# AnnaLew/pangenomix

Hardware: AMD Instinct MI355X
Metric: proteins/sec clustered at 0.8 identity + pan/core iters/sec, 400-genome set (higher is better)
Workload: dtype i32

## Files before the change

### pangenomix_amd/csrc/cluster.hip

```cpp
#include <algorithm>
#include <chrono>
#include <cstdlib>
#include <cmath>
#include <type_traits>
#include <functional>
#include <condition_variable>
#include <mutex>
#include <thread>
#include <vector>

#include "cluster_layout.h"
#include "cluster_tables.h"
#include "pgx_internal.h"

namespace {

using namespace pgxc;

constexpr uint32_t kWindowMax = 65536;
constexpr int kDiscoveryRounds = 2;
constexpr uint32_t kBlockCap = 4096;
constexpr uint32_t kBlockCapMin = 64;

constexpr uint32_t kMaxLen = 1u << 22;
constexpr uint32_t kPackedLenAa = 32767, kPackedLenNt = 16383;
constexpr uint32_t kSentinel = 0xFFFFFFFFu;
constexpr uint32_t kDiagLdsCap = 2048;
constexpr uint32_t kDiagLdsSmall = 512;
constexpr int kMaxBand = 64;

__constant__ int8_t kBlosum62_dev[kNAA1 * kNAA1] = PGXC_BLOSUM62_FLAT;

enum : uint32_t { F_DIAG_PASS = 1, F_BAND_OK = 2, F_ACCEPT = 4, F_TOO_BIG = 8, F_EVAL = 16, F_ALIGNED = 32 };
// ... 43 lines not shown
    const uint32_t *wcode;
    const uint16_t *wmult;
    const uint32_t *wcnt;
    const uint32_t *pk;
    const uint32_t *pk_off;
    uint32_t n_fwd;
    int32_t base;
    int32_t kd;
    int32_t nt;
    uint32_t mshift;
};
__device__ __forceinline__ uint32_t entry_rmask(const DevSeqs &S) { return (1u << S.mshift) - 1u; }
__device__ __forceinline__ uint32_t entry_fmax(const DevSeqs &S) { return 0xFFFFFFFFu >> S.mshift; }
__device__ __forceinline__ uint32_t real_of(const DevSeqs &S, uint32_t k) { return k >= S.n_fwd ? k - S.n_fwd : k; }

__constant__ int8_t kAa2Idx_dev[26] = {0, 2, 4, 3, 6, 13, 7, 8, 9, 20, 11, 10, 12,
                                       2, 20, 14, 5, 1, 15, 16, 20, 19, 17, 20, 18, 6};

__device__ __forceinline__ bool is_letter(uint8_t ch) {
    ch &= 0xDF;
    return ch >= 'A' && ch <= 'Z';
}

__global__ __launch_bounds__(256) void seq_len_kernel(const uint8_t *__restrict__ res,
                                                     const uint64_t *__restrict__ off, uint32_t n, uint64_t total,
                                                     uint32_t *__restrict__ len) {
    const uint32_t lane = threadIdx.x & 63u;
    const uint32_t i = blockIdx.x * 4u + (threadIdx.x >> 6);
    if (i >= n) return;
    const uint64_t b = off[i], e = off[i + 1];
    uint32_t c = 0;
    const uint64_t a0 = b & ~3ull;
    for (uint64_t a = a0 + 4ull * lane; a < e; a += 256) {
        uint32_t word = 0;
        if (a + 4 <= total) word = *reinterpret_cast<const uint32_t *>(res + a);
        else for (uint64_t p = a; p < total; ++p) word |= (uint32_t)res[p] << (8 * (p - a));
#pragma unroll
        for (int t = 0; t < 4; ++t) {
            const uint64_t p = a + t;
            c += (p >= b && p < e) && is_letter((uint8_t)(word >> (8 * t)));
        }
    }
    for (int d = 32; d > 0; d >>= 1) c += __shfl_xor(c, d);
    if (lane == 0) len[i] = c;
}

__global__ __launch_bounds__(256) void encode_gather_kernel(const uint8_t *__restrict__ in,
                                                           const uint64_t *__restrict__ in_off,
                                                           const uint32_t *__restrict__ order,
                                                           const uint64_t *__restrict__ out_off,
                                                           uint8_t *__restrict__ out, uint32_t n, int nt) {
    const uint32_t lane = threadIdx.x & 63u;
    const uint32_t k = blockIdx.x * 4u + (threadIdx.x >> 6);
    if (k >= n) return;
    const uint32_t src = order[k];
    const uint64_t b = in_off[src], e = in_off[src + 1];
    uint64_t w = out_off[k];
    for (uint64_t q0 = b; q0 < e; q0 += 256) {
        uint8_t chs[4];
#pragma unroll
        for (int j = 0; j < 4; ++j) { const uint64_t p = q0 + 64u * j + lane; chs[j] = p < e ? in[p] : (uint8_t)0; }
#pragma unroll
        for (int j = 0; j < 4; ++j) {
            const uint8_t ch = chs[j];
            const bool ok = is_letter(ch);
            const unsigned long long m = __ballot(ok);
            if (ok) {
                const uint8_t up = ch & 0xDF;
                const uint8_t idx = nt ? (uint8_t)(up == 'A' ? 0 : up == 'C' ? 1 : up == 'G' ? 2 : (up == 'T' || up == 'U') ? 3 : 4)
                                       : (uint8_t)kAa2Idx_dev[up - 'A'];
                out[w + __popcll(m & ((1ull << lane) - 1ull))] = idx;
            }
            w += __popcll(m);
        }
    }
}

__global__ __launch_bounds__(256) void revcomp_kernel(uint8_t *__restrict__ res, const uint64_t *__restrict__ off,
                                                     const uint32_t *__restrict__ len, uint32_t n) {
    const uint32_t lane = threadIdx.x & 63u;
    const uint32_t k = blockIdx.x * 4u + (threadIdx.x >> 6);
    if (k >= n) return;
    const uint64_t src = off[k], dst = off[n + k];
    const uint32_t L = len[k];
    for (uint32_t i = lane; i < L; i += 64) {
        const uint8_t b = res[src + L - 1 - i];
        res[dst + i] = b < 4 ? (uint8_t)(3 - b) : b;
    }
}

__global__ __launch_bounds__(256) void pack5_kernel(const uint8_t *__restrict__ res, const uint64_t *__restrict__ off,
                                                   const uint32_t *__restrict__ len,
                                                   const uint32_t *__restrict__ pk_off, uint32_t n,
                                                   uint32_t *__restrict__ pk) {
    const uint32_t lane = threadIdx.x & 63u;
    const uint32_t k = blockIdx.x * 4u + (threadIdx.x >> 6);
    if (k >= n) return;
    const uint8_t *s = res + off[k];
    const uint32_t L = len[k], nw = (L + 5u) / 6u;
    uint32_t *dst = pk + pk_off[k];
    for (uint32_t w = lane; w < nw; w += 64) {
        uint32_t x = 0;
        for (uint32_t t = 0; t < 6; ++t)
            if (6 * w + t < L) x |= (uint32_t)s[6 * w + t] << (5u * t);
        dst[w] = x;
    }
}

constexpr uint32_t kDevSortMaxLen = 65535;
constexpr uint32_t kHistLds = 4096;
constexpr uint32_t kSortShare = 1024;
constexpr uint32_t kSortCells = 4u << 20;
constexpr uint32_t kScanTile = 2048;
enum : uint32_t { H_OVER = 0, H_MAX = 1, H_BINS = 4 };

constexpr int kClearSegs = 6;
struct ClearArgs { uint32_t *p[kClearSegs]; uint32_t words[kClearSegs]; int n; uint32_t *one; };
__global__ __launch_bounds__(256) void clear_kernel(ClearArgs a) {
    const uint32_t t = blockIdx.x * 256u + threadIdx.x, step = gridDim.x * 256u;
    for (int s = 0; s < a.n; ++s)
        for (uint32_t i = t; i < a.words[s]; i += step) a.p[s][i] = 0u;
    if (a.one && t == 0) *a.one = 1u;
}

__global__ __launch_bounds__(1024) void len_hist_kernel(const uint32_t *__restrict__ len, uint32_t n, int32_t min_length,
                                                       uint32_t *__restrict__ hist) {
    __shared__ uint32_t h[kHistLds];
    for (uint32_t b = threadIdx.x; b < kHistLds; b += 1024u) h[b] = 0u;
// ... 1926 lines not shown
    S.n_input = n_in;
    if (out_n_clusters) *out_n_clusters = 0;
    const unsigned nth = host_threads(n_in);
    parallel_for(n_in, nth, [&](unsigned, size_t b, size_t e) {
        for (size_t i = b; i < e; ++i) {
            out_cluster[i] = -1; out_member[i] = -1; out_identity[i] = 0.f;
            if (out_strand) out_strand[i] = 0;
        }
    });
    if (n_in == 0) { if (stats) *stats = S; return PGX_OK; }

    DevBuf d_res(ctx, CL_SLOT_RES), d_off(ctx, CL_SLOT_OFF), d_len(ctx, CL_SLOT_LEN), d_wcode(ctx, CL_SLOT_WCODE),
        d_wmult(ctx, CL_SLOT_WMULT), d_wcnt(ctx, CL_SLOT_WCNT), d_aa1(ctx, CL_SLOT_AA1), d_aas(ctx, CL_SLOT_AAS),
        d_aan(ctx, CL_SLOT_AAN), d_lines(ctx, CL_SLOT_LINES), d_pool[2] = {{ctx, CL_SLOT_POOL0}, {ctx, CL_SLOT_POOL1}},
        d_idx(ctx, CL_SLOT_IDX), d_newbits(ctx, CL_SLOT_NEWBITS), d_touched(ctx, CL_SLOT_TOUCHED), d_first(ctx, CL_SLOT_FIRST),
        d_best_own(ctx, CL_SLOT_BEST_OWN), d_rcvis(ctx, CL_SLOT_RCVIS), d_counters(ctx, CL_SLOT_COUNTERS),
        d_visits(ctx, CL_SLOT_VISITS), d_pairsW(ctx, CL_SLOT_PAIRS_W), d_pairsK(ctx, CL_SLOT_PAIRS_K),
        d_blk_list(ctx, CL_SLOT_BLK_LIST), d_ulist(ctx, CL_SLOT_ULIST), d_new_list(ctx, CL_SLOT_NEW_LIST),
        d_flags(ctx, CL_SLOT_FLAGS), d_gscratch(ctx, CL_SLOT_GSCRATCH), d_order(ctx, CL_SLOT_ORDER), d_list(ctx, CL_SLOT_LIST),
        d_gather(ctx, CL_SLOT_GATHER), d_pk(ctx, CL_SLOT_PK), d_pkoff(ctx, CL_SLOT_PKOFF),
        d_counters2(ctx, CL_SLOT_COUNTERS2), d_best2(ctx, CL_SLOT_BEST2), d_flags2(ctx, CL_SLOT_FLAGS2),
        d_pairsW2(ctx, CL_SLOT_PAIRS_W2), d_gscratch2(ctx, CL_SLOT_GSCRATCH2),
        d_thr(ctx, CL_SLOT_THR), d_hugewords(ctx, CL_SLOT_HUGEWORDS), d_xsend(ctx, CL_SLOT_XSEND), d_xrecv(ctx, CL_SLOT_XRECV),
        d_hist(ctx, CL_SLOT_HIST), d_sortcnt(ctx, CL_SLOT_SORTCNT), d_tilesum(ctx, CL_SLOT_TILESUM), d_runs(ctx, CL_SLOT_RUNS);
    uint32_t n_codes = 1;
    for (int t = 0; t < P->word_len; ++t) n_codes *= nt ? 4u : (uint32_t)kNAA1;
    static_assert(kSegs == 4, "eight codes per word of the round's map");
    const uint32_t bm_words = (n_codes / 8 + 2 + 3) & ~3u;
    const bool overlap = !nt && !std::getenv("PGX_NO_OVERLAP");
    DevBuf d_in_len(ctx, CL_SLOT_IN_LEN);
    PGX_HIP(d_in_len.alloc((size_t)n_in * 4));
    constexpr uint32_t kHistWords = H_BINS + kDevSortMaxLen + 1;
    PGX_HIP(d_hist.alloc((size_t)kHistWords * 4));
    PGX_HIP(d_idx.alloc(16));
    PGX_HIP(d_newbits.alloc(2 * (size_t)bm_words * 4 + 16));
    PGX_HIP(d_counters.alloc(C_COUNT * 4));
    PGX_HIP(d_visits.alloc(8));
    if (overlap) PGX_HIP(d_counters2.alloc(C_COUNT * 4));
    {
        ClearArgs ca{};
        auto seg = [&](DevBuf &b, size_t words) { ca.p[ca.n] = b.as<uint32_t>(); ca.words[ca.n] = (uint32_t)words; ++ca.n; };
        seg(d_hist, kHistWords);
        seg(d_newbits, 2 * (size_t)bm_words);
        seg(d_counters, C_COUNT);
        seg(d_visits, 2);
        if (overlap) seg(d_counters2, C_COUNT);
        ca.one = d_idx.as<uint32_t>();
        clear_kernel<<<1024, 256, 0, st>>>(ca);
        LAUNCH_CHECK();
    }
    {
        ProfScope prof(ctx, "seq_len_kernel", st);
        seq_len_kernel<<<(n_in + 3) / 4, 256, 0, st>>>(d_residues, d_offsets, n_in, total_in, d_in_len.as<uint32_t>());
        len_hist_kernel<<<std::min(64u, (n_in + 1023u) / 1024u), 1024, 0, st>>>(d_in_len.as<uint32_t>(), n_in, P->min_length,
                                                                               d_hist.as<uint32_t>());
    }
    LAUNCH_CHECK();
    HostVec<uint32_t> h_hist(ctx, CL_HOST_HIST, kHistWords);
    PGX_REQUIRE(h_hist.ok(), "out of host memory");
    PGX_HIP(hipMemcpyAsync(h_hist.data(), d_hist.p, (size_t)(H_BINS + kHistLds) * 4, hipMemcpyDeviceToHost, st));
    PGX_HIP(hipStreamSynchronize(st));
    const bool dev_sort = h_hist[H_OVER] == 0 && !std::getenv("PGX_HOST_PROLOGUE");
    uint32_t max_len = h_hist[H_MAX];
    if (dev_sort && max_len >= kHistLds) {
        PGX_HIP(hipMemcpyAsync(h_hist.data() + H_BINS + kHistLds, d_hist.as<uint32_t>() + H_BINS + kHistLds,
                               (size_t)(max_len + 1 - kHistLds) * 4, hipMemcpyDeviceToHost, st));
        PGX_HIP(hipStreamSynchronize(st));
    }
    phase("  seq_len + histogram + copy");
    const uint32_t *len_hist = h_hist.data() + H_BINS;
    uint32_t n = 0;
    HostVec<uint32_t> order(ctx, CL_HOST_ORDER, dev_sort ? 0 : n_in);
    std::vector<uint32_t> host_hist;
    if (dev_sort) {
        for (uint32_t L = 0; L <= max_len; ++L) n += len_hist[L];
    } else {
// ... 179 lines not shown
        ca.p[0] = cnt; ca.words[0] = cells; ca.n = 1;
        clear_kernel<<<std::min(2048u, (cells + 255u) / 256u), 256, 0, st>>>(ca);
        sort_count_kernel<<<(n_in + 255) / 256, 256, 0, st>>>(in_len, n_in, P->min_length, max_len, per, n_shares, cnt);
        tile_sum_kernel<<<tiles, 256, 0, st>>>(cnt, cells, d_tilesum.as<uint32_t>());
        tile_scan_kernel<<<tiles, 256, 0, st>>>(cnt, cells, d_tilesum.as<uint32_t>());
        sort_place_kernel<<<(n_shares + 3) / 4, 256, 0, st>>>(in_len, n_in, P->min_length, max_len, per, n_shares, cnt, n,
                                                              d_order.as<uint32_t>());
        LAUNCH_CHECK();
        PGX_HIP(hipMemcpyAsync(order.data(), d_order.p, (size_t)n * 4, hipMemcpyDeviceToHost, st));
    } else {
        PGX_HIP(hipMemcpyAsync(d_order.p, order.data(), (size_t)n * 4, hipMemcpyHostToDevice, st));
    }
    {
        const size_t runs_bytes = 2 * ((size_t)n_runs + 1) * 8;
        PGX_HIP(d_runs.alloc(runs_bytes));
        PGX_HIP(hipMemcpyAsync(d_runs.p, h_runs.data(), runs_bytes, hipMemcpyHostToDevice, st));
        const uint64_t *const dr_off = d_runs.as<uint64_t>();
        const uint32_t *const dr_pos = reinterpret_cast<const uint32_t *>(dr_off + n_runs + 1), *const dr_pk = dr_pos + n_runs + 1;
        layout_kernel<<<nv / 256 + 1, 256, 0, st>>>(dr_off, dr_pos, dr_pk, n_runs, max_len, n, nv, d_len.as<uint32_t>(),
                                                    d_off.as<uint64_t>(), d_pkoff.as<uint32_t>());
        LAUNCH_CHECK();
    }
    {
        ProfScope prof(ctx, "encode_gather_kernel", st);
        encode_gather_kernel<<<(n + 3) / 4, 256, 0, st>>>(d_residues, d_offsets, d_order.as<uint32_t>(),
                                                          d_off.as<uint64_t>(), d_res.as<uint8_t>(), n, nt ? 1 : 0);
        if (both)
            revcomp_kernel<<<(n + 3) / 4, 256, 0, st>>>(d_res.as<uint8_t>(), d_off.as<uint64_t>(),
                                                        d_len.as<uint32_t>(), n);
        pack5_kernel<<<(nv + 3) / 4, 256, 0, st>>>(d_res.as<uint8_t>(), d_off.as<uint64_t>(), d_len.as<uint32_t>(),
                                                   d_pkoff.as<uint32_t>(), nv, d_pk.as<uint32_t>());
    }
    LAUNCH_CHECK();
    {
        PGX_HIP(d_thr.alloc(3 * ((size_t)max_len + 1) * 4));
        PGX_HIP(hipMemcpyAsync(d_thr.p, h_thr.data(), 3 * ((size_t)max_len + 1) * 4, hipMemcpyHostToDevice, st));
        thresholds_kernel<<<(n + 255) / 256, 256, 0, st>>>(d_len.as<uint32_t>(), n, d_thr.as<int32_t>(), max_len + 1,
                                                          d_aa1.as<int32_t>(), d_aas.as<int32_t>(), d_aan.as<int32_t>());
        LAUNCH_CHECK();
    }
    phase("alloc + sort + layout + encode (enq)");
    {
        const int wl = P->word_len;
        auto first_with_words_le = [&](uint32_t cap) { return pgxc::first_with_words_le(run_pos, max_len, cap, wl); };
        const uint32_t k32 = first_with_words_le(32768), k8 = first_with_words_le(8192),
                       k2 = first_with_words_le(2048), k1k = first_with_words_le(1023), k5 = first_with_words_le(512);
        int rc;
        uint8_t *r8 = d_res.as<uint8_t>(); uint64_t *o64 = d_off.as<uint64_t>(); uint32_t *l32 = d_len.as<uint32_t>();
        uint32_t *wc = d_wcode.as<uint32_t>(); uint16_t *wm = d_wmult.as<uint16_t>(); uint32_t *wn = d_wcnt.as<uint32_t>();
        const int base = nt ? 4 : kNAA1;
        for (uint32_t half = 0; half < (both ? 2u : 1u); ++half) {
            const uint32_t o = half * n;
            if (k32) {
                uint32_t slots = 65536;
// ... 34 lines not shown
    phase("host lengths + offsets");
    uint64_t max_window_words = 0;
    uint32_t max_chunks = 1;
    {
        Chunks C;
        size_t nf = 0;
        for (uint32_t b0 = 0, nbw; b0 < n; b0 += nbw) {
            while (nf < flush_at.size() && flush_at[nf] <= b0) ++nf;
            nbw = form_window(b0, C, nf < flush_at.size() ? flush_at[nf] : n);
            max_window_words = std::max<uint64_t>(max_window_words, h_off[b0 + nbw] - h_off[b0]);
            max_chunks = std::max(max_chunks, C.n);
        }
        if (!flush_at.empty())
            max_window_words = std::max<uint64_t>(max_window_words, h_off[std::min(n, window_cap)]);
    }
    if (chunking && flush_at.empty())
        max_window_words = std::max<uint64_t>(max_window_words,
            std::min<uint64_t>(h_off[std::min(n, window_cap)], (uint64_t)kMaxChunks * std::max<uint64_t>(chunk_words, max_len)));
    PGX_REQUIRE(max_window_words < 0xFFFFFFF0ull, "window too large");
    PGX_HIP(d_touched.alloc((max_window_words + 16) * sizeof(Deferred)));
    if (chunking && n > window_cap / 2) max_chunks = kMaxChunks;
    uint32_t tag_stride = 1;
    while (tag_stride < max_chunks) tag_stride *= 2;
    PGX_HIP(d_first.alloc((size_t)tag_stride * n_codes * 4 + 16));
    std::vector<uint32_t> rep_seq;
    HostVec<int32_t> cluster_of(ctx, CL_HOST_CLUSTER_OF, n, -1);
    HostVec<int32_t> iden_of(ctx, CL_HOST_IDEN_OF, n, -1);
    PGX_REQUIRE(cluster_of.ok() && iden_of.ok(), "out of host memory");
    Pinned<Pair> hW(ctx, CL_PIN_W), hK(ctx, CL_PIN_K);
    Pinned<unsigned long long> h_best(ctx, CL_PIN_BEST), h_rcvis(ctx, CL_PIN_RCVIS);
    Pinned<uint32_t> h_cnt(ctx, CL_PIN_CNT), h_blk(ctx, CL_PIN_BLK), h_new(ctx, CL_PIN_NEW), h_list(ctx, CL_PIN_LIST),
        h_push(ctx, CL_PIN_PUSH);
    Pinned<Pair> h_gather(ctx, CL_PIN_GATHER);
    constexpr uint32_t kPrefix = 65536;
    PGX_HIP(h_best.reserve(window_cap)); PGX_HIP(h_cnt.reserve(C_COUNT)); PGX_HIP(h_blk.reserve(kBlockCap));
    PGX_HIP(h_new.reserve(window_cap)); PGX_HIP(hK.reserve(pair_cap_k)); PGX_HIP(hW.reserve(kPrefix));
    PGX_HIP(h_rcvis.reserve(window_cap)); PGX_HIP(h_push.reserve(2 * (size_t)window_cap + 4 * kBlockCap));
    PGX_HIP(h_list.reserve(pair_cap_k)); PGX_HIP(h_gather.reserve(pair_cap_k));
    Pinned<Pair> hW2(ctx, CL_PIN_W2);
    Pinned<unsigned long long> h_best2(ctx, CL_PIN_BEST2);
    Pinned<uint32_t> h_ccnt(ctx, CL_PIN_CCNT), h_ccnt2(ctx, CL_PIN_CCNT2);
    PGX_HIP(h_ccnt.reserve(C_COUNT));
    if (overlap) { PGX_HIP(hW2.reserve(kPrefix)); PGX_HIP(h_best2.reserve(window_cap)); PGX_HIP(h_ccnt2.reserve(C_COUNT)); }
    struct Events {
        hipEvent_t strike[2] = {nullptr, nullptr}, post[2] = {nullptr, nullptr};
        ~Events() { for (hipEvent_t e : strike) if (e) (void)hipEventDestroy(e); for (hipEvent_t e : post) if (e) (void)hipEventDestroy(e); }
    } ev;
// ... 32 lines not shown
    uint64_t n_rounds = 0;

    uint64_t gpu_pairs = 0, gpu_aligned = 0, gpu_aligned_bytes = 0, filter_walk_words = 0;
    auto account = [&](const Pair *pp, uint32_t cnt) {
        for (uint32_t i = 0; i < cnt; ++i) {
            ++gpu_pairs;
            if ((pp[i].flags & (F_DIAG_PASS | F_BAND_OK)) != (F_DIAG_PASS | F_BAND_OK)) continue;
            ++gpu_aligned;
            gpu_aligned_bytes += h_len[pp[i].q] + h_len[pp[i].r];
        }
    };
    auto window_error = [&](uint32_t e, uint32_t at) {
        pgx_set_error("pgx_cluster_greedy: capacity failure in the window at %u%s:%s%s%s%s%s%s", at,
                      exchanging ? " (on this or another process)" : "",
                      e & E_TOUCHED ? " append scratch list full;" : "", e & E_POOL ? " overflow pool of the word index full;" : "",
                      e & E_TABLE ? " exact table of the filter overflowed;" : "",
                      e & E_BAND ? " alignment band wider than 64 diagonals;" : "", e & E_PAIRS ? " candidate pair buffer overflow;" : "",
                      e & E_WORDMULT ? " a word occurs more than 65535 times in one sequence;" : "");
    };
    const bool trace = std::getenv("PGX_TRACE") != nullptr;
    const uint32_t filter_grid = 4096u;
    uint32_t epoch_idx = 0;
    uint32_t epoch_tag = 0;
    PGX_HIP(hipMemsetAsync(d_first.p, 0, (size_t)tag_stride * n_codes * 4, st));
    phase("window set-up");
    const auto t_loop0 = std::chrono::steady_clock::now();
    double t_resolve = 0.0, t_close = 0.0;
    uint64_t n_blocks = 0;
    g_wait_s = 0.0;
    std::function<int()> deferred;
    std::vector<uint32_t> members;
    uint64_t pending_words = 0;
    Chunks chunks;
    Pinned<uint8_t> h_taken(ctx, CL_PIN_TAKEN);
    if (!flush_at.empty()) { PGX_HIP(h_taken.reserve(n)); std::fill(h_taken.p, h_taken.p + n, (uint8_t)0); }
    auto drain = [&]() -> int {
        if (deferred) { int rc = deferred(); deferred = nullptr; if (rc) return rc; }
        PGX_HIP(hipStreamSynchronize(st_main));
        PGX_HIP(hipStreamSynchronize(ctx->stream2));
        return PGX_OK;
    };
    size_t next_flush = 0;
    bool sweeping = false;
    uint32_t sweep_at = 0;
    for (uint32_t cursor = 0, nb = 0; cursor < n;) {
        if (!sweeping && next_flush < flush_at.size() && cursor == flush_at[next_flush]) {
            ++next_flush;
// ... 146 lines not shown
            LAUNCH_CHECK();
            return PGX_OK;
        };
        auto filter_new_and_evaluate = [&](const uint32_t *d_lo, const uint32_t *d_hi) -> int {
            FilterArgs F = FA;
            F.epoch = epoch_idx; F.d_round_lo = d_lo; F.d_round_hi = d_hi;
            F.newbits = d_newbits.as<uint32_t>() + (size_t)(epoch_idx & 1u) * bm_words;
            {
                ProfScope prof(ctx, "filter_kernel<new>", st);
                auto kern = nt ? filter_kernel<true, true> : filter_kernel<false, true>;
                kern<<<std::min(filter_grid, (ns + 3) / 4), 256, 0, st>>>(DS, F);
            }
            LAUNCH_CHECK();
            filter_walk_words += window_words * (both ? 2 : 1) / shard_count;
            return evaluate_round();
        };
        uint32_t n_listed = 0;
        if (sweep) { int rc = begin_host_side(); if (rc) return rc; }
        if (!sweep) {
        if (overlap && S.sweeps > 1)
            PGX_HIP(hipStreamWaitEvent(st, ev.post[set ^ 1], 0));
        static const int n_disc = std::getenv("PGX_ROUNDS") ? std::atoi(std::getenv("PGX_ROUNDS")) : kDiscoveryRounds;
        for (int round = 0; round < n_disc; ++round) {
            if (++epoch_tag == 0xFFFFu) { PGX_HIP(hipMemsetAsync(d_first.p, 0, (size_t)tag_stride * n_codes * 4, st)); epoch_tag = 1; }
            const uint32_t which = (uint32_t)round & 1u;
            uint32_t *const d_n_open = dc + (which ? C_ROUND_OPEN2 : C_ROUND_OPEN);
            list_open_kernel<<<(nb + 255) / 256, 256, 0, st>>>(d_best, d_done, b0, nb, d_ulist.as<uint32_t>(), dc, which);
            LAUNCH_CHECK();
            {
                ProfScope prof(ctx, "discover_kernels", st);
                first_open_kernel<<<std::min(2048u, (nb + 3) / 4), 256, 0, st>>>(DS, d_ulist.as<uint32_t>(), d_n_open, b0,
                                                                                 epoch_tag, d_first.as<uint32_t>(), tag_stride,
                                                                                 chunks, d_aan.as<int32_t>(), d_accepted);
                certain_kernel<<<std::min(2048u, (nb + 3) / 4), 256, 0, st>>>(DS, d_ulist.as<uint32_t>(), d_n_open, b0,
                                                                              both ? 1u : 0u, epoch_tag, d_first.as<uint32_t>(), tag_stride,
                                                                              chunks,
                                                                              d_aan.as<int32_t>(), d_accepted, d_done, d_new_list.as<uint32_t>(),
                                                                              dc + C_NEW);
            }
            LAUNCH_CHECK();
            int rc = index_append(d_new_list.as<uint32_t>(), dc + C_SEG0, dc + C_NEW);
            if (rc) return rc;
            rc = filter_new_and_evaluate(dc + C_SEG0, dc + C_NEW);
            if (rc) return rc;
        }
        bool first_block = true;
        n_listed = 0;
// ... 318 lines not shown
        unsigned long long h[16], z[16] = {0};
        PGX_HIP(hipMemcpyFromSymbol(h, HIP_SYMBOL(g_ftime), sizeof h));
        PGX_HIP(hipMemcpyToSymbol(HIP_SYMBOL(g_ftime), z, sizeof z));
        static const char *nm[12] = {"prologue", "words+probes", "compaction", "last slab", "sync+reduce", "pass2 begin",
                                     "pass2 walk", "pass2 sync", "emit", "bucket clear", "kernel end", "-"};
        double tot = 0;
        for (int i = 0; i < 12; ++i) tot += (double)h[i];
        for (int i = 0; i < 11; ++i) fprintf(stderr, "[ftime] %-14s %6.2f %%\n", nm[i], 100.0 * (double)h[i] / tot);
        fprintf(stderr, "[ftime] %llu waves, %.0f clocks per wave; direct %llu, fallbacks %llu, classic %llu\n", h[12], tot / (double)h[12], h[13], h[14], h[15]);
    }
#endif
    if (overlap) PGX_HIP(hipStreamSynchronize(ctx->stream2));
    unsigned long long visits_table = 0;
    PGX_HIP(hipMemcpyAsync(&visits_table, d_visits.p, 8, hipMemcpyDeviceToHost, st));
    PGX_HIP(hipStreamSynchronize(st));
    S.posting_visits = visits_table + visits_rc;
    S.reserved[0] = gpu_pairs; S.reserved[1] = gpu_aligned; S.reserved[2] = gpu_aligned_bytes;
    S.reserved[3] = filter_walk_words;
    S.n_clusters = rep_seq.size();

    phase("window loop");
    if (out_n_clusters) *out_n_clusters = (uint32_t)rep_seq.size();
    if (stats) *stats = S;
    return PGX_OK;
}

extern "C" int pgx_cluster_greedy(pgx_ctx *ctx, const uint8_t *residues, const uint64_t *offsets,
                                  uint32_t n_in, const pgx_cluster_params *P, int32_t *out_cluster,
                                  int32_t *out_member, float *out_identity, uint8_t *out_strand,
                                  uint32_t *out_n_clusters, pgx_cluster_stats *stats) {
    PGX_REQUIRE(ctx && P, "NULL argument");
    PGX_REQUIRE(n_in == 0 || (residues && offsets), "NULL sequence arrays");
    PGX_HIP(hipSetDevice(ctx->device_id));
    for (uint32_t i = 0; i < n_in; ++i) PGX_REQUIRE(offsets[i + 1] >= offsets[i], "offsets must be non-decreasing");
    const uint64_t total_in = n_in ? offsets[n_in] : 0;
    DevBuf d_res(ctx, CL_SLOT_UP_RES), d_off(ctx, CL_SLOT_UP_OFF);
    PGX_HIP(d_res.alloc(total_in + 16));
    PGX_HIP(d_off.alloc(((size_t)n_in + 1) * 8));
    if (n_in) {
        { int rc = pgx_staged_h2d(ctx, d_res.p, residues, total_in, ctx->stream); if (rc) return rc; }
        PGX_HIP(hipMemcpyAsync(d_off.p, offsets, ((size_t)n_in + 1) * 8, hipMemcpyHostToDevice, ctx->stream));
    }
    return pgx_cluster_greedy_dev(ctx, d_res.as<uint8_t>(), d_off.as<uint64_t>(), n_in, total_in, P, out_cluster,
                                  out_member, out_identity, out_strand, out_n_clusters, stats, ctx->stream);
}
```

### pangenomix_amd/csrc/pgx_internal.h

```cpp
#pragma once
#include <hip/hip_runtime.h>
#include <cstdarg>
#include <cstdint>
#include <cstdio>
#include <cstring>
#include "../../include/pgx.h"
#include "pgx_guard.h"
#include "pgx_pack.h"

#include <string>
#include <utility>
#include <algorithm>
#include <cstdlib>
#include <vector>

struct ProfSlot {
    std::string name;
    double total_ms = 0.0;
    uint64_t launches = 0;
    std::vector<std::pair<hipEvent_t, hipEvent_t>> pending;
};

enum DevSlot : int {
    CL_SLOT_IN_LEN = 0, CL_SLOT_RES, CL_SLOT_OFF, CL_SLOT_LEN, CL_SLOT_WCODE, CL_SLOT_WMULT, CL_SLOT_WCNT, CL_SLOT_AA1,
    CL_SLOT_AAS, CL_SLOT_AAN, CL_SLOT_LINES, CL_SLOT_POOL0, CL_SLOT_POOL1, CL_SLOT_IDX, CL_SLOT_NEWBITS, CL_SLOT_TOUCHED,
    CL_SLOT_FIRST, CL_SLOT_BEST_OWN, CL_SLOT_RCVIS, CL_SLOT_COUNTERS, CL_SLOT_VISITS, CL_SLOT_PAIRS_W, CL_SLOT_PAIRS_K,
    CL_SLOT_BLK_LIST, CL_SLOT_ULIST, CL_SLOT_NEW_LIST, CL_SLOT_FLAGS, CL_SLOT_GSCRATCH, CL_SLOT_ORDER, CL_SLOT_LIST,
    CL_SLOT_GATHER, CL_SLOT_PK, CL_SLOT_PKOFF, CL_SLOT_COUNTERS2, CL_SLOT_BEST2, CL_SLOT_FLAGS2, CL_SLOT_PAIRS_W2,
    CL_SLOT_GSCRATCH2, CL_SLOT_THR, CL_SLOT_HUGEWORDS, CL_SLOT_XSEND, CL_SLOT_XRECV, CL_SLOT_HIST, CL_SLOT_SORTCNT,
    CL_SLOT_TILESUM, CL_SLOT_RUNS, CL_SLOT_UP_RES, CL_SLOT_UP_OFF,
    PC_SLOT_ROWS, PC_SLOT_GENOMES, PC_SLOT_BITS, PC_SLOT_PERMS, PC_SLOT_PAN, PC_SLOT_CORE, PC_SLOT_WS, PC_SLOT_CNT,
    PC_SLOT_COUNTS, PC_SLOT_TABLE, PGX_SLOT_RESIDENT, PC_SLOT_RES_A, PC_SLOT_RES_B, PC_SLOT_RES_C, PC_SLOT_RES_D,
    HP_SLOT_TAB, HP_SLOT_A, HP_SLOT_K,
    PGX_SLOT_BERN_BITS, BN_SLOT_ROWS, BN_SLOT_GENOMES, BN_SLOT_CNT, BN_SLOT_MAP, BN_SLOT_PQ, BN_SLOT_OUT, BN_SLOT_WS,
    BB_SLOT_WORDS0, BB_SLOT_WORDS1, BB_SLOT_CDF, BB_SLOT_MODEL, BB_SLOT_KS, BB_SLOT_HIST, BB_SLOT_IDX,
    FC_SLOT_BITS, FC_SLOT_ROWS, FC_SLOT_GENOMES, FC_SLOT_CNT, FC_SLOT_WS, FC_SLOT_MAP, FC_SLOT_CMAP, FC_SLOT_CROWS,
    FC_SLOT_CCOLS, FC_SLOT_CLEARED,
    FC_SLOT_M_LISTS, FC_SLOT_M_WS, FC_SLOT_M_OUT, FC_SLOT_M_MATRIX,
    AS_SLOT_BITS, AS_SLOT_ROWS, AS_SLOT_GENOMES, AS_SLOT_CNT, AS_SLOT_WS, AS_SLOT_IN, AS_SLOT_OUT,
    RN_SLOT_ABITS, RN_SLOT_AROWS, RN_SLOT_AGENOMES, RN_SLOT_ACNT, RN_SLOT_GBITS, RN_SLOT_GROWS, RN_SLOT_GGENOMES,
    RN_SLOT_GCNT, RN_SLOT_IN, RN_SLOT_WS, RN_SLOT_OUT,
    CS_SLOT_WS, CS_SLOT_THR, CS_SLOT_OUT,
    SC_SLOT_TEXT, SC_SLOT_KEYS, SC_SLOT_FOUND, SC_SLOT_WS,
    CD_SLOT_INIT, CD_SLOT_TABLE, CD_SLOT_SOLVER, CD_SLOT_WS,
    DM_SLOT_KEYS, DM_SLOT_KEY_OFF, DM_SLOT_TABLE, DM_SLOT_QUERIES, DM_SLOT_QUERY_OFF, DM_SLOT_OUT,
    SD_SLOT_ROWS, SD_SLOT_GENOMES, SD_SLOT_A_BITS, SD_SLOT_A_CNT, SD_SLOT_B_BITS, SD_SLOT_B_CNT, SD_SLOT_OUT,
    SV_SLOT_BITS, SV_SLOT_ROWS, SV_SLOT_GENOMES, SV_SLOT_CNT, SV_SLOT_WS, SV_SLOT_IN, SV_SLOT_OUT,
    PX_SLOT_TEXT, PX_SLOT_WINDOWS, PX_SLOT_OUT, PX_SLOT_BLOB, PX_SLOT_RECORDS, PX_SLOT_WS, PX_SLOT_RESULT,
    AN_SLOT_TOK, AN_SLOT_OFFSETS, AN_SLOT_WS, AN_SLOT_RESULT,
    GR_SLOT_IN, GR_SLOT_WS, GR_SLOT_OUT,
    TS_SLOT_TEXT, TS_SLOT_IN, TS_SLOT_OUT,
    DEV_SLOT_COUNT
};
// ... 9 lines not shown
    SV_HOST_STATUS,
    PX_HOST_OFFSETS,
    HOST_SLOT_COUNT
};
enum PinSlot : int {
    CL_PIN_W = 0, CL_PIN_K, CL_PIN_BEST, CL_PIN_CNT, CL_PIN_BLK, CL_PIN_NEW, CL_PIN_RCVIS, CL_PIN_LIST, CL_PIN_GATHER,
    CL_PIN_PUSH, CL_PIN_W2, CL_PIN_BEST2, CL_PIN_CCNT, CL_PIN_CCNT2, CL_PIN_TAKEN,
    PIN_SLOT_COUNT
};

struct pgx_ctx {
    int device_id;
    hipStream_t stream;
    hipStream_t stream2;
    hipEvent_t ev_main = nullptr, ev_side[2] = {nullptr, nullptr};
    hipDeviceProp_t prop;
    bool profiling = false;
    std::vector<ProfSlot> prof;
    std::vector<hipEvent_t> event_pool;
    std::pair<void *, size_t> arena[DEV_SLOT_COUNT] = {};
    std::pair<void *, size_t> host_arena[PIN_SLOT_COUNT] = {};
    std::pair<void *, size_t> host_scratch[HOST_SLOT_COUNT] = {};
    std::vector<hipEvent_t> stage_events;
    uint64_t resident_token = 0, resident_next = 1;
    uint32_t resident_genes = 0, resident_genomes = 0;
    uint32_t bern_genes = 0, bern_genomes = 0;
    bool bern_loaded = false;
    uint64_t bern_cd_stats[4] = {0, 0, 0, 0};
    bool dict_loaded = false;
    uint32_t dict_keys = 0, dict_flags = 0;
    const void *dict_d_keys = nullptr, *dict_d_offsets = nullptr, *dict_d_table = nullptr;
    std::vector<int32_t> fcd_rows, fcd_cols;
    std::vector<uint64_t> fcd_row_off, fcd_col_off, fcd_left;
    void *comm = nullptr;
    int comm_rank = 0, comm_world = 0;
};

template <typename T>
struct HostVec {
    T *p = nullptr;
    size_t n = 0;
    HostVec(pgx_ctx *ctx, HostSlot slot, size_t count) { bind(ctx, slot, count); }
    HostVec(pgx_ctx *ctx, HostSlot slot, size_t count, T fill) {
        bind(ctx, slot, count);
        if (p) std::fill(p, p + n, fill);
    }
// ... 195 lines not shown
```

Before: 16.45 million.

## Fuse encode and 5-bit packing into length-bucketed SWAR kernel; cache tag epoch

Replaces the per-sequence wave-wide encode_gather and pack5 passes with a fused encode_pack kernel. It reads 16-byte chunks, encodes four residues per word through byte-permute table lookups, and writes both the byte codes and the 5-bit packed words. Sequences are split into length buckets and handled by thread groups of 64, 16 or 8, and sequences containing non-letter characters go to a slow-path list that the old kernels handle. seq_len now counts letters with SWAR over 16-thread groups. The tag buffer memset is skipped across calls by carrying the epoch tag in the context, which reuses state between calls and relies on the buffer staying untouched.

```diff
diff --git a/pangenomix_amd/csrc/cluster.hip b/pangenomix_amd/csrc/cluster.hip
--- a/pangenomix_amd/csrc/cluster.hip
+++ b/pangenomix_amd/csrc/cluster.hip
@@ -9,6 +9,7 @@
 #include <thread>
 #include <vector>
 
+#include "cluster_encode.h"
 #include "cluster_layout.h"
 #include "cluster_tables.h"
 #include "pgx_internal.h"
@@ -98,56 +99,150 @@
     return ch >= 'A' && ch <= 'Z';
 }
 
+struct Bytes16 { uint32_t w[4]; };
+struct __attribute__((packed, aligned(1))) Packed16 { uint32_t w[4]; };
+struct __attribute__((packed, aligned(1))) Packed8 { uint64_t v; };
+struct __attribute__((packed, aligned(1))) Packed4 { uint32_t v; };
+struct __attribute__((packed, aligned(1))) Packed2 { uint16_t v; };
+struct __attribute__((packed, aligned(4))) Words4 { uint32_t w[4]; };
+__device__ __forceinline__ Bytes16 load16(const uint8_t *__restrict__ in, uint64_t at, uint64_t lo, uint64_t hi) {
+    Bytes16 r;
+    if (at >= lo && at + 16 <= hi) {
+        const Packed16 x = *reinterpret_cast<const Packed16 *>(in + at);
+        r.w[0] = x.w[0]; r.w[1] = x.w[1]; r.w[2] = x.w[2]; r.w[3] = x.w[3];
+    } else {
+        r.w[0] = r.w[1] = r.w[2] = r.w[3] = 0u;
+        for (uint32_t t = 0; t < 16; ++t)
+            if (at + t >= lo && at + t < hi) r.w[t >> 2] |= (uint32_t)in[at + t] << (8u * (t & 3u));
+    }
+    return r;
+}
+
+constexpr uint32_t kLenGroup = 16;
 __global__ __launch_bounds__(256) void seq_len_kernel(const uint8_t *__restrict__ res,
                                                      const uint64_t *__restrict__ off, uint32_t n, uint64_t total,
                                                      uint32_t *__restrict__ len) {
-    const uint32_t lane = threadIdx.x & 63u;
-    const uint32_t i = blockIdx.x * 4u + (threadIdx.x >> 6);
+    const uint32_t gl = threadIdx.x & (kLenGroup - 1u);
+    const uint32_t i = (blockIdx.x * 256u + threadIdx.x) / kLenGroup;
     if (i >= n) return;
-    const uint64_t b = off[i], e = off[i + 1];
+    const uint64_t mis = reinterpret_cast<uintptr_t>(res) & 15u;
+    const uint8_t *const base = res - mis;
+    const uint64_t b = mis + off[i], e = mis + off[i + 1];
     uint32_t c = 0;
-    const uint64_t a0 = b & ~3ull;
-    for (uint64_t a = a0 + 4ull * lane; a < e; a += 256) {
-        uint32_t word = 0;
-        if (a + 4 <= total) word = *reinterpret_cast<const uint32_t *>(res + a);
-        else for (uint64_t p = a; p < total; ++p) word |= (uint32_t)res[p] << (8 * (p - a));
+    for (uint64_t a = (b & ~15ull) + 16ull * gl; a < e; a += 32ull * kLenGroup) {
+        const uint64_t a2 = a + 16ull * kLenGroup;
+        Bytes16 x = load16(base, a, mis, mis + total), y;
+        if (a2 < e) y = load16(base, a2, mis, mis + total);
+        else y.w[0] = y.w[1] = y.w[2] = y.w[3] = 0u;
+        if (b > a) drop_first(x.w, 4, (uint32_t)(b - a));
+        if (e - a < 16) keep_first(x.w, 4, (uint32_t)(e - a));
+        if (a2 < e && e - a2 < 16) keep_first(y.w, 4, (uint32_t)(e - a2));
 #pragma unroll
-        for (int t = 0; t < 4; ++t) {
-            const uint64_t p = a + t;
-            c += (p >= b && p < e) && is_letter((uint8_t)(word >> (8 * t)));
-        }
-    }
-    for (int d = 32; d > 0; d >>= 1) c += __shfl_xor(c, d);
-    if (lane == 0) len[i] = c;
+        for (int t = 0; t < 4; ++t) c += __popc(letter_bits(x.w[t])) + __popc(letter_bits(y.w[t]));
+    }
+    for (int d = kLenGroup / 2; d > 0; d >>= 1) c += __shfl_xor(c, d);
+    if (gl == 0) len[i] = c;
+}
+
+constexpr uint32_t kEncLen8 = 8u * kLaneBytes, kEncLen16 = 16u * kLaneBytes;
+template <uint32_t G>
+__global__ __launch_bounds__(256) void encode_pack_kernel(const uint8_t *__restrict__ in,
+                                                         const uint64_t *__restrict__ in_off, uint64_t total,
+                                                         const uint32_t *__restrict__ order,
+                                                         const uint64_t *__restrict__ out_off,
+                                                         const uint32_t *__restrict__ len,
+                                                         const uint32_t *__restrict__ pk_off, uint32_t k0, uint32_t k1,
+                                                         EncTable T, uint8_t *__restrict__ out,
+                                                         uint32_t *__restrict__ pk, uint32_t *__restrict__ slow) {
+    const uint32_t gl = threadIdx.x & (G - 1u);
+    const uint32_t k = k0 + (blockIdx.x * 256u + threadIdx.x) / G;
+    if (k >= k1) return;
+    const uint32_t src = order[k], L = len[k];
+    const uint64_t b = in_off[src], e = in_off[src + 1];
+    if (e - b != (uint64_t)L) {
+        if (gl == 0) slow[1u + atomicAdd(slow, 1u)] = k;
+        return;
+    }
+    uint8_t *const dst = out + out_off[k];
+    uint32_t *const dpk = pk + pk_off[k];
+    for (uint32_t p = gl * kLaneBytes; p < L; p += G * kLaneBytes) {
+        const uint32_t rem = L - p;
+        uint32_t enc[kLaneWords];
+#pragma unroll
+        for (int j = 0; j < 3; ++j) {
+            Bytes16 x;
+            if (rem > 16u * j) x = load16(in, b + p + 16u * j, 0, total);
+            else x.w[0] = x.w[1] = x.w[2] = x.w[3] = 0u;
+#pragma unroll
+            for (int t = 0; t < 4; ++t) enc[4 * j + t] = encode4(x.w[t], T);
+        }
+        if (rem < kLaneBytes) keep_first(enc, (int)kLaneWords, rem);
+#pragma unroll
+        for (int j = 0; j < 3; ++j) {
+            uint8_t *q = dst + p + 16u * j;
+            if (rem >= 16u * (j + 1)) {
+                Packed16 s;
+#pragma unroll
+                for (int t = 0; t < 4; ++t) s.w[t] = enc[4 * j + t];
+                *reinterpret_cast<Packed16 *>(q) = s;
+            } else if (rem > 16u * j) {
+                const uint32_t r = rem - 16u * j;
+                uint64_t cur = enc[4 * j] | (uint64_t)enc[4 * j + 1] << 32;
+                if (r & 8u) {
+                    reinterpret_cast<Packed8 *>(q)->v = cur;
+                    cur = enc[4 * j + 2] | (uint64_t)enc[4 * j + 3] << 32; q += 8;
+                }
+                if (r & 4u) { reinterpret_cast<Packed4 *>(q)->v = (uint32_t)cur; cur >>= 32; q += 4; }
+                if (r & 2u) { reinterpret_cast<Packed2 *>(q)->v = (uint16_t)cur; cur >>= 16; q += 2; }
+                if (r & 1u) *q = (uint8_t)cur;
+            }
+        }
+        uint32_t w[kLanePacked];
+        pack48(enc, w);
+        uint32_t *const qw = dpk + p / 6u;
+        const uint32_t nw = rem >= kLaneBytes ? kLanePacked : (rem + 5u) / 6u;
+        if (nw == kLanePacked) {
+            Words4 s0, s1;
+#pragma unroll
+            for (int t = 0; t < 4; ++t) { s0.w[t] = w[t]; s1.w[t] = w[4 + t]; }
+            *reinterpret_cast<Words4 *>(qw) = s0;
+            *reinterpret_cast<Words4 *>(qw + 4) = s1;
+        } else {
+#pragma unroll
+            for (int t = 0; t < (int)kLanePacked - 1; ++t)
+                if ((uint32_t)t < nw) qw[t] = w[t];
+        }
+    }
 }
 
 __global__ __launch_bounds__(256) void encode_gather_kernel(const uint8_t *__restrict__ in,
                                                            const uint64_t *__restrict__ in_off,
                                                            const uint32_t *__restrict__ order,
                                                            const uint64_t *__restrict__ out_off,
-                                                           uint8_t *__restrict__ out, uint32_t n, int nt) {
-    const uint32_t lane = threadIdx.x & 63u;
-    const uint32_t k = blockIdx.x * 4u + (threadIdx.x >> 6);
-    if (k >= n) return;
-    const uint32_t src = order[k];
-    const uint64_t b = in_off[src], e = in_off[src + 1];
-    uint64_t w = out_off[k];
-    for (uint64_t q0 = b; q0 < e; q0 += 256) {
-        uint8_t chs[4];
+                                                           uint8_t *__restrict__ out, const uint32_t *__restrict__ slow, int nt) {
+    const uint32_t lane = threadIdx.x & 63u, n = slow[0];
+    for (uint32_t i = blockIdx.x * 4u + (threadIdx.x >> 6); i < n; i += gridDim.x * 4u) {
+        const uint32_t k = slow[1u + i];
+        const uint32_t src = order[k];
+        const uint64_t b = in_off[src], e = in_off[src + 1];
+        uint64_t w = out_off[k];
+        for (uint64_t q0 = b; q0 < e; q0 += 256) {
+            uint8_t chs[4];
 #pragma unroll
-        for (int j = 0; j < 4; ++j) { const uint64_t p = q0 + 64u * j + lane; chs[j] = p < e ? in[p] : (uint8_t)0; }
+            for (int j = 0; j < 4; ++j) { const uint64_t p = q0 + 64u * j + lane; chs[j] = p < e ? in[p] : (uint8_t)0; }
 #pragma unroll
-        for (int j = 0; j < 4; ++j) {
-            const uint8_t ch = chs[j];
-            const bool ok = is_letter(ch);
-            const unsigned long long m = __ballot(ok);
-            if (ok) {
-                const uint8_t up = ch & 0xDF;
-                const uint8_t idx = nt ? (uint8_t)(up == 'A' ? 0 : up == 'C' ? 1 : up == 'G' ? 2 : (up == 'T' || up == 'U') ? 3 : 4)
-                                       : (uint8_t)kAa2Idx_dev[up - 'A'];
-                out[w + __popcll(m & ((1ull << lane) - 1ull))] = idx;
-            }
-            w += __popcll(m);
+            for (int j = 0; j < 4; ++j) {
+                const uint8_t ch = chs[j];
+                const bool ok = is_letter(ch);
+                const unsigned long long m = __ballot(ok);
+                if (ok) {
+                    const uint8_t up = ch & 0xDF;
+                    const uint8_t idx = nt ? (uint8_t)(up == 'A' ? 0 : up == 'C' ? 1 : up == 'G' ? 2 : (up == 'T' || up == 'U') ? 3 : 4)
+                                           : (uint8_t)kAa2Idx_dev[up - 'A'];
+                    out[w + __popcll(m & ((1ull << lane) - 1ull))] = idx;
+                }
+                w += __popcll(m);
+            }
         }
     }
 }
@@ -167,19 +262,21 @@
 
 __global__ __launch_bounds__(256) void pack5_kernel(const uint8_t *__restrict__ res, const uint64_t *__restrict__ off,
                                                    const uint32_t *__restrict__ len,
-                                                   const uint32_t *__restrict__ pk_off, uint32_t n,
-                                                   uint32_t *__restrict__ pk) {
+                                                   const uint32_t *__restrict__ pk_off, const uint32_t *__restrict__ slow,
+                                                   uint32_t k0, uint32_t n, uint32_t *__restrict__ pk) {
     const uint32_t lane = threadIdx.x & 63u;
-    const uint32_t k = blockIdx.x * 4u + (threadIdx.x >> 6);
-    if (k >= n) return;
-    const uint8_t *s = res + off[k];
-    const uint32_t L = len[k], nw = (L + 5u) / 6u;
-    uint32_t *dst = pk + pk_off[k];
-    for (uint32_t w = lane; w < nw; w += 64) {
-        uint32_t x = 0;
-        for (uint32_t t = 0; t < 6; ++t)
-            if (6 * w + t < L) x |= (uint32_t)s[6 * w + t] << (5u * t);
-        dst[w] = x;
+    if (slow) n = slow[0];
+    for (uint32_t i = blockIdx.x * 4u + (threadIdx.x >> 6); i < n; i += gridDim.x * 4u) {
+        const uint32_t k = slow ? slow[1u + i] : k0 + i;
+        const uint8_t *s = res + off[k];
+        const uint32_t L = len[k], nw = (L + 5u) / 6u;
+        uint32_t *dst = pk + pk_off[k];
+        for (uint32_t w = lane; w < nw; w += 64) {
+            uint32_t x = 0;
+            for (uint32_t t = 0; t < 6; ++t)
+                if (6 * w + t < L) x |= (uint32_t)s[6 * w + t] << (5u * t);
+            dst[w] = x;
+        }
     }
 }
 
@@ -2152,7 +2249,8 @@
         d_counters2(ctx, CL_SLOT_COUNTERS2), d_best2(ctx, CL_SLOT_BEST2), d_flags2(ctx, CL_SLOT_FLAGS2),
         d_pairsW2(ctx, CL_SLOT_PAIRS_W2), d_gscratch2(ctx, CL_SLOT_GSCRATCH2),
         d_thr(ctx, CL_SLOT_THR), d_hugewords(ctx, CL_SLOT_HUGEWORDS), d_xsend(ctx, CL_SLOT_XSEND), d_xrecv(ctx, CL_SLOT_XRECV),
-        d_hist(ctx, CL_SLOT_HIST), d_sortcnt(ctx, CL_SLOT_SORTCNT), d_tilesum(ctx, CL_SLOT_TILESUM), d_runs(ctx, CL_SLOT_RUNS);
+        d_hist(ctx, CL_SLOT_HIST), d_sortcnt(ctx, CL_SLOT_SORTCNT), d_tilesum(ctx, CL_SLOT_TILESUM), d_runs(ctx, CL_SLOT_RUNS),
+        d_slow(ctx, CL_SLOT_SLOW);
     uint32_t n_codes = 1;
     for (int t = 0; t < P->word_len; ++t) n_codes *= nt ? 4u : (uint32_t)kNAA1;
     static_assert(kSegs == 4, "eight codes per word of the round's map");
@@ -2167,6 +2265,7 @@
     PGX_HIP(d_counters.alloc(C_COUNT * 4));
     PGX_HIP(d_visits.alloc(8));
     if (overlap) PGX_HIP(d_counters2.alloc(C_COUNT * 4));
+    PGX_HIP(d_slow.alloc(((size_t)n_in + 1) * 4));
     {
         ClearArgs ca{};
         auto seg = [&](DevBuf &b, size_t words) { ca.p[ca.n] = b.as<uint32_t>(); ca.words[ca.n] = (uint32_t)words; ++ca.n; };
@@ -2175,13 +2274,14 @@
         seg(d_counters, C_COUNT);
         seg(d_visits, 2);
         if (overlap) seg(d_counters2, C_COUNT);
+        seg(d_slow, 1);
         ca.one = d_idx.as<uint32_t>();
         clear_kernel<<<1024, 256, 0, st>>>(ca);
         LAUNCH_CHECK();
     }
     {
         ProfScope prof(ctx, "seq_len_kernel", st);
-        seq_len_kernel<<<(n_in + 3) / 4, 256, 0, st>>>(d_residues, d_offsets, n_in, total_in, d_in_len.as<uint32_t>());
+        seq_len_kernel<<<(n_in + 256 / kLenGroup - 1) / (256 / kLenGroup), 256, 0, st>>>(d_residues, d_offsets, n_in, total_in, d_in_len.as<uint32_t>());
         len_hist_kernel<<<std::min(64u, (n_in + 1023u) / 1024u), 1024, 0, st>>>(d_in_len.as<uint32_t>(), n_in, P->min_length,
                                                                                d_hist.as<uint32_t>());
     }
@@ -2407,14 +2507,39 @@
         LAUNCH_CHECK();
     }
     {
-        ProfScope prof(ctx, "encode_gather_kernel", st);
-        encode_gather_kernel<<<(n + 3) / 4, 256, 0, st>>>(d_residues, d_offsets, d_order.as<uint32_t>(),
-                                                          d_off.as<uint64_t>(), d_res.as<uint8_t>(), n, nt ? 1 : 0);
-        if (both)
-            revcomp_kernel<<<(n + 3) / 4, 256, 0, st>>>(d_res.as<uint8_t>(), d_off.as<uint64_t>(),
-                                                        d_len.as<uint32_t>(), n);
-        pack5_kernel<<<(nv + 3) / 4, 256, 0, st>>>(d_res.as<uint8_t>(), d_off.as<uint64_t>(), d_len.as<uint32_t>(),
-                                                   d_pkoff.as<uint32_t>(), nv, d_pk.as<uint32_t>());
+        ProfScope prof(ctx, "encode_pack_kernel", st);
+        EncTable tab{};
+        for (uint32_t c = 0; c < 26; ++c) {
+            const char up = (char)('A' + c);
+            const uint32_t idx = nt ? (up == 'A' ? 0u : up == 'C' ? 1u : up == 'G' ? 2u : (up == 'T' || up == 'U') ? 3u : 4u)
+                                    : (uint32_t)kAa2Idx[c];
+            tab.t[c >> 2] |= idx << (8u * (c & 3u));
+        }
+        const uint32_t k16 = max_len > kEncLen16 ? run_pos[max_len - kEncLen16] : 0u, k8 = max_len > kEncLen8 ? run_pos[max_len - kEncLen8] : 0u;
+        uint8_t *const r8 = d_res.as<uint8_t>();
+        uint32_t *const pk32 = d_pk.as<uint32_t>(), *const slow = d_slow.as<uint32_t>();
+        if (k16)
+            encode_pack_kernel<64><<<(k16 + 3) / 4, 256, 0, st>>>(d_residues, d_offsets, total_in, d_order.as<uint32_t>(),
+                                                                  d_off.as<uint64_t>(), d_len.as<uint32_t>(), d_pkoff.as<uint32_t>(),
+                                                                  0u, k16, tab, r8, pk32, slow);
+        if (k8 > k16)
+            encode_pack_kernel<16><<<(k8 - k16 + 15) / 16, 256, 0, st>>>(d_residues, d_offsets, total_in, d_order.as<uint32_t>(),
+                                                                        d_off.as<uint64_t>(), d_len.as<uint32_t>(), d_pkoff.as<uint32_t>(),
+                                                                        k16, k8, tab, r8, pk32, slow);
+        if (n > k8)
+            encode_pack_kernel<8><<<(n - k8 + 31) / 32, 256, 0, st>>>(d_residues, d_offsets, total_in, d_order.as<uint32_t>(),
+                                                                     d_off.as<uint64_t>(), d_len.as<uint32_t>(), d_pkoff.as<uint32_t>(),
+                                                                     k8, n, tab, r8, pk32, slow);
+        const uint32_t slow_grid = std::min(256u, (n + 3) / 4);
+        encode_gather_kernel<<<slow_grid, 256, 0, st>>>(d_residues, d_offsets, d_order.as<uint32_t>(), d_off.as<uint64_t>(), r8,
+                                                        slow, nt ? 1 : 0);
+        if (both) {
+            revcomp_kernel<<<(n + 3) / 4, 256, 0, st>>>(r8, d_off.as<uint64_t>(), d_len.as<uint32_t>(), n);
+            pack5_kernel<<<std::min(2048u, (n + 3) / 4), 256, 0, st>>>(r8, d_off.as<uint64_t>(), d_len.as<uint32_t>(),
+                                                                       d_pkoff.as<uint32_t>(), nullptr, n, n, pk32);
+        }
+        pack5_kernel<<<slow_grid, 256, 0, st>>>(r8, d_off.as<uint64_t>(), d_len.as<uint32_t>(), d_pkoff.as<uint32_t>(), slow,
+                                                0u, 0u, pk32);
     }
     LAUNCH_CHECK();
     {
@@ -2495,7 +2620,8 @@
     if (chunking && n > window_cap / 2) max_chunks = kMaxChunks;
     uint32_t tag_stride = 1;
     while (tag_stride < max_chunks) tag_stride *= 2;
-    PGX_HIP(d_first.alloc((size_t)tag_stride * n_codes * 4 + 16));
+    const size_t tag_bytes = (size_t)tag_stride * n_codes * 4;
+    PGX_HIP(d_first.alloc(tag_bytes + 16));
     std::vector<uint32_t> rep_seq;
     HostVec<int32_t> cluster_of(ctx, CL_HOST_CLUSTER_OF, n, -1);
     HostVec<int32_t> iden_of(ctx, CL_HOST_IDEN_OF, n, -1);
@@ -2574,7 +2700,15 @@
     const uint32_t filter_grid = 4096u;
     uint32_t epoch_idx = 0;
     uint32_t epoch_tag = 0;
-    PGX_HIP(hipMemsetAsync(d_first.p, 0, (size_t)tag_stride * n_codes * 4, st));
+    {
+        const auto &slot = ctx->arena[CL_SLOT_FIRST];
+        if (ctx->cl_tag_bytes == tag_bytes && ctx->cl_tag_stride == tag_stride && ctx->cl_tag_buf == slot.first &&
+            ctx->cl_tag_cap == slot.second)
+            epoch_tag = ctx->cl_tag_epoch;
+        else
+            PGX_HIP(hipMemsetAsync(d_first.p, 0, tag_bytes, st));
+        ctx->cl_tag_bytes = 0;
+    }
     phase("window set-up");
     const auto t_loop0 = std::chrono::steady_clock::now();
     double t_resolve = 0.0, t_close = 0.0;
@@ -2767,7 +2901,7 @@
             PGX_HIP(hipStreamWaitEvent(st, ev.post[set ^ 1], 0));
         static const int n_disc = std::getenv("PGX_ROUNDS") ? std::atoi(std::getenv("PGX_ROUNDS")) : kDiscoveryRounds;
         for (int round = 0; round < n_disc; ++round) {
-            if (++epoch_tag == 0xFFFFu) { PGX_HIP(hipMemsetAsync(d_first.p, 0, (size_t)tag_stride * n_codes * 4, st)); epoch_tag = 1; }
+            if (++epoch_tag == 0xFFFFu) { PGX_HIP(hipMemsetAsync(d_first.p, 0, tag_bytes, st)); epoch_tag = 1; }
             const uint32_t which = (uint32_t)round & 1u;
             uint32_t *const d_n_open = dc + (which ? C_ROUND_OPEN2 : C_ROUND_OPEN);
             list_open_kernel<<<(nb + 255) / 256, 256, 0, st>>>(d_best, d_done, b0, nb, d_ulist.as<uint32_t>(), dc, which);
@@ -3132,6 +3266,8 @@
     phase("window loop");
     if (out_n_clusters) *out_n_clusters = (uint32_t)rep_seq.size();
     if (stats) *stats = S;
+    ctx->cl_tag_buf = ctx->arena[CL_SLOT_FIRST].first; ctx->cl_tag_cap = ctx->arena[CL_SLOT_FIRST].second;
+    ctx->cl_tag_bytes = tag_bytes; ctx->cl_tag_stride = tag_stride; ctx->cl_tag_epoch = epoch_tag;
     return PGX_OK;
 }
 
diff --git a/pangenomix_amd/csrc/cluster_encode.h b/pangenomix_amd/csrc/cluster_encode.h
--- /dev/null
+++ b/pangenomix_amd/csrc/cluster_encode.h
@@ -0,0 +1,72 @@
+#pragma once
+#include <cstdint>
+
+#if defined(__HIPCC__)
+#define PGXC_HD __attribute__((host)) __attribute__((device)) inline __attribute__((always_inline))
+#else
+#define PGXC_HD inline
+#endif
+
+namespace pgxc {
+
+constexpr uint32_t kLaneBytes = 48, kLaneWords = kLaneBytes / 4, kLanePacked = kLaneBytes / 6;
+
+PGXC_HD uint32_t letter_bits(uint32_t x) {
+    const uint32_t u = x & 0xDFDFDFDFu, t = u & 0x7F7F7F7Fu;
+    return (t + 0x3F3F3F3Fu) & ~(t + 0x25252525u) & ~u & 0x80808080u;
+}
+
+PGXC_HD uint32_t pick_bytes(uint32_t hi, uint32_t lo, uint32_t sel) {
+#if defined(__HIP_DEVICE_COMPILE__)
+    return __builtin_amdgcn_perm(hi, lo, sel);
+#else
+    const uint64_t tab = ((uint64_t)hi << 32) | lo;
+    uint32_t r = 0;
+    for (int i = 0; i < 4; ++i) r |= (uint32_t)((tab >> (8u * ((sel >> (8 * i)) & 7u))) & 0xFFu) << (8 * i);
+    return r;
+#endif
+}
+
+struct EncTable { uint32_t t[8]; };
+
+PGXC_HD uint32_t encode4(uint32_t x, const EncTable &T) {
+    const uint32_t c = (x & 0xDFDFDFDFu) - 0x41414141u;
+    const uint32_t sel = c & 0x07070707u;
+    const uint32_t by3 = ((c >> 1) & 0x04040404u) | 0x03020100u, by4 = ((c >> 2) & 0x04040404u) | 0x03020100u;
+    const uint32_t r0 = pick_bytes(T.t[1], T.t[0], sel), r1 = pick_bytes(T.t[3], T.t[2], sel);
+    const uint32_t r2 = pick_bytes(T.t[5], T.t[4], sel), r3 = pick_bytes(T.t[7], T.t[6], sel);
+    return pick_bytes(pick_bytes(r3, r2, by3), pick_bytes(r1, r0, by3), by4);
+}
+
+PGXC_HD void keep_first(uint32_t *e, int n, uint32_t rem) {
+    const uint32_t full = rem >> 2, part = (1u << (8u * (rem & 3u))) - 1u;
+#if defined(__HIP_DEVICE_COMPILE__)
+#pragma unroll
+#endif
+    for (int t = 0; t < n; ++t) e[t] = (uint32_t)t < full ? e[t] : (uint32_t)t == full ? e[t] & part : 0u;
+}
+PGXC_HD void drop_first(uint32_t *e, int n, uint32_t skip) {
+    const uint32_t full = skip >> 2, part = (1u << (8u * (skip & 3u))) - 1u;
+#if defined(__HIP_DEVICE_COMPILE__)
+#pragma unroll
+#endif
+    for (int t = 0; t < n; ++t) e[t] = (uint32_t)t < full ? 0u : (uint32_t)t == full ? e[t] & ~part : e[t];
+}
+
+PGXC_HD uint32_t squeeze4(uint32_t e) {
+    const uint32_t t = (e & 0x001F001Fu) | ((e & 0x1F001F00u) >> 3);
+    return (t & 0x3FFu) | ((t >> 6) & 0xFFC00u);
+}
+
+PGXC_HD void pack48(const uint32_t e[kLaneWords], uint32_t w[kLanePacked]) {
+#if defined(__HIP_DEVICE_COMPILE__)
+#pragma unroll
+#endif
+    for (int g = 0; g < 4; ++g) {
+        const uint32_t q0 = squeeze4(e[3 * g]), q1 = squeeze4(e[3 * g + 1]), q2 = squeeze4(e[3 * g + 2]);
+        w[2 * g] = q0 | ((q1 & 0x3FFu) << 20);
+        w[2 * g + 1] = (q1 >> 10) | (q2 << 10);
+    }
+}
+
+}
diff --git a/pangenomix_amd/csrc/pgx_internal.h b/pangenomix_amd/csrc/pgx_internal.h
--- a/pangenomix_amd/csrc/pgx_internal.h
+++ b/pangenomix_amd/csrc/pgx_internal.h
@@ -28,7 +28,7 @@
     CL_SLOT_BLK_LIST, CL_SLOT_ULIST, CL_SLOT_NEW_LIST, CL_SLOT_FLAGS, CL_SLOT_GSCRATCH, CL_SLOT_ORDER, CL_SLOT_LIST,
     CL_SLOT_GATHER, CL_SLOT_PK, CL_SLOT_PKOFF, CL_SLOT_COUNTERS2, CL_SLOT_BEST2, CL_SLOT_FLAGS2, CL_SLOT_PAIRS_W2,
     CL_SLOT_GSCRATCH2, CL_SLOT_THR, CL_SLOT_HUGEWORDS, CL_SLOT_XSEND, CL_SLOT_XRECV, CL_SLOT_HIST, CL_SLOT_SORTCNT,
-    CL_SLOT_TILESUM, CL_SLOT_RUNS, CL_SLOT_UP_RES, CL_SLOT_UP_OFF,
+    CL_SLOT_TILESUM, CL_SLOT_RUNS, CL_SLOT_SLOW, CL_SLOT_UP_RES, CL_SLOT_UP_OFF,
     PC_SLOT_ROWS, PC_SLOT_GENOMES, PC_SLOT_BITS, PC_SLOT_PERMS, PC_SLOT_PAN, PC_SLOT_CORE, PC_SLOT_WS, PC_SLOT_CNT,
     PC_SLOT_COUNTS, PC_SLOT_TABLE, PGX_SLOT_RESIDENT, PC_SLOT_RES_A, PC_SLOT_RES_B, PC_SLOT_RES_C, PC_SLOT_RES_D,
     HP_SLOT_TAB, HP_SLOT_A, HP_SLOT_K,
@@ -84,6 +84,9 @@
     std::pair<void *, size_t> host_arena[PIN_SLOT_COUNT] = {};
     std::pair<void *, size_t> host_scratch[HOST_SLOT_COUNT] = {};
     std::vector<hipEvent_t> stage_events;
+    void *cl_tag_buf = nullptr;
+    size_t cl_tag_cap = 0, cl_tag_bytes = 0;
+    uint32_t cl_tag_stride = 0, cl_tag_epoch = 0;
     uint64_t resident_token = 0, resident_next = 1;
     uint32_t resident_genes = 0, resident_genomes = 0;
     uint32_t bern_genes = 0, bern_genomes = 0;
```

After: 16.76 million (median of 6 runs). +1.9%, better.
